# thrill/thrill

Hardware: AMD Instinct MI355X
Metric: TeraSort keys/sec (100-byte recs) (higher is better)
Workload: dtype u8; 1 GPU; terasort_10GiB_100B; records=107374182, record_bytes=100, seed=0x7421, parallelism=dp1

## Files before the change

thrill_amd/csrc/t9_bitonic.h:

```cpp
#pragma once
#include "t9_common.h"

__device__ inline void t9_ce_xor(u64& c, u32& v, u32 lanemask, bool lower,
                                 bool asc) {
    const u64 oc = __shfl_xor(c, lanemask);
    const u32 ov = __shfl_xor(v, lanemask);
    if ((c > oc) == (lower == asc)) { c = oc; v = ov; }
}

template <int SUBMAX, int BLOCK, bool HAS_VAL>
__global__ __launch_bounds__(BLOCK, 2) void k_bitonic_sort_sub(
    u64* __restrict__ keys, u32* __restrict__ vals,
    const u32* __restrict__ sub_start, const u32* __restrict__ sub_n) {
    constexpr int E = SUBMAX / BLOCK;
    static_assert(E == 4, "mapping assumes 4 elements per thread");
    __shared__ u64 s_c[SUBMAX];
    __shared__ u32 s_v[HAS_VAL ? SUBMAX : 1];
    __shared__ u32 s_differ;

    const u32 sb = blockIdx.x;
    const u32 ns = sub_n[sb];
    if (ns <= 1 || ns > (u32)SUBMAX) return;
    const u32 gbase = sub_start[sb];
    const u32 tid = threadIdx.x, lane = tid & 63;

    if (tid == 0) s_differ = 0;
    __syncthreads();

    const u64 mask48 = 0x0000FFFFFFFFFFFFull;
    const u64 high16 = keys[gbase] & ~mask48;
    const u64 ref48 = keys[gbase] & mask48;

    u64 c[E];
    u32 v[E];
    u32 differ = 0;
    const u32 e0 = tid * E;
#pragma unroll
    for (int r = 0; r < E; ++r) {
        const u32 i = e0 + r;
        if (i < ns) {
            const u64 k = keys[gbase + i];
            c[r] = ((k & mask48) << 12) | (u64)i;
            if (HAS_VAL) v[r] = vals[gbase + i];
            differ |= ((k & mask48) != ref48);
        } else {
            c[r] = ~0ull;
            if (HAS_VAL) v[r] = 0;
        }
    }
    if (differ) s_differ = 1;
    __syncthreads();
    if (!s_differ) return;

    constexpr int LOG = (SUBMAX == 1024) ? 10 : (SUBMAX == 2048) ? 11 : 12;
// ... 39 lines not shown
                        const bool asc = ((e0 + r) & k) == 0;
                        if ((c[r] > c[q]) == asc) {
                            u64 tc = c[r]; c[r] = c[q]; c[q] = tc;
                            if (HAS_VAL) {
                                u32 tv = v[r]; v[r] = v[q]; v[q] = tv;
                            }
                        }
                    }
                }
            }
        }
    }

#pragma unroll
    for (int r = 0; r < E; ++r) {
        const u32 i = e0 + r;
        if (i < ns) {
            keys[gbase + i] = high16 | (c[r] >> 12);
            if (HAS_VAL) vals[gbase + i] = v[r];
        }
    }
}

typedef unsigned long long t9_u64x2 __attribute__((ext_vector_type(2)));

__device__ __forceinline__ u32 t9_w16_phys(u32 e) {
    return e ^ (((e >> 4) & 7u) << 1);
}

__device__ __forceinline__ void t9_w16_row_store(u64* lc, u32 row,
                                                 const u64 (&c)[16]) {
    const u32 base = row * 16 + ((row & 7u) << 1);
#pragma unroll
    for (int k = 0; k < 8; ++k) {
        t9_u64x2 v2;
        v2.x = c[2 * k];
        v2.y = c[2 * k + 1];
        *(t9_u64x2*)&lc[base ^ ((u32)k << 1)] = v2;
    }
}

__device__ __forceinline__ void t9_w16_row_load(const u64* lc, u32 row,
                                                u64 (&c)[16]) {
    const u32 base = row * 16 + ((row & 7u) << 1);
#pragma unroll
    for (int k = 0; k < 8; ++k) {
        const t9_u64x2 v2 = *(const t9_u64x2*)&lc[base ^ ((u32)k << 1)];
        c[2 * k] = v2.x;
        c[2 * k + 1] = v2.y;
    }
}

template <int NSORT, int BLOCK, bool HAS_VAL, bool REC>
__global__ __launch_bounds__(BLOCK, 2) void k_wave16_sort_sub(
    u64* __restrict__ keys, u32* __restrict__ vals,
    const u32* __restrict__ sub_start, const u32* __restrict__ sub_n,
    u32* __restrict__ ntied) {
    constexpr int E = NSORT / BLOCK;
    static_assert(E == 16, "wave16 mapping: 16 elements per lane");
    static_assert(HAS_VAL || !REC, "the tie count rides the pair sort");
    constexpr int ROUNDS = (NSORT == 1024) ? 6 : (NSORT == 2048) ? 7 : 8;
    __shared__ __attribute__((aligned(16))) u64 lc[NSORT];
    __shared__ u32 s_differ;
    __shared__ u32 s_ntie;

    const u32 sb = blockIdx.x;
    const u32 ns = sub_n[sb];
    if (ns <= 1 || ns > (u32)NSORT) return;
    const u32 gbase = sub_start[sb];
    const u32 lane = threadIdx.x;
    const u32 e0 = lane * E;

    if (lane == 0) { s_differ = 0; s_ntie = 0; }
    __syncthreads();

    const u64 mask48 = 0x0000FFFFFFFFFFFFull;
    const u64 high16 = keys[gbase] & ~mask48;
    const u64 ref48 = keys[gbase] & mask48;

    u64 c[E];
    u32 differ = 0;
    u64* const kb = keys + gbase;
    u32* const vb = HAS_VAL ? vals + gbase : nullptr;
#pragma unroll
    for (int r = 0; r < E; ++r) {
        const u32 p = lane + (u32)BLOCK * r;
        u64 cc = ~0ull;
        if (p < ns) {
            const u64 k = kb[p];
            cc = ((k & mask48) << 12) | (u64)p;
            differ |= ((k & mask48) != ref48);
        }
        lc[t9_w16_phys(p)] = cc;
    }
    if (differ) s_differ = 1;
    __syncthreads();
    if (!s_differ) {
        if (REC && lane == 0) atomicAdd(ntied, ns - 1);
        return;
    }
    t9_w16_row_load(lc, lane, c);

#pragma unroll
    for (int lk = 1; lk <= 4; ++lk) {
        const int k = 1 << lk;
#pragma unroll
        for (int lj = lk - 1; lj >= 0; --lj) {
            const int j = 1 << lj;
#pragma unroll
            for (int r = 0; r < E; ++r) {
                const int q = r ^ j;
                if (q > r) {
                    const bool asc = (r & k) == 0;
                    if ((c[r] > c[q]) == asc) {
                        u64 tc = c[r]; c[r] = c[q]; c[q] = tc;
                    }
                }
            }
        }
// ... 30 lines not shown
                ia += ta ? 1u : 0u;
                ib += ta ? 0u : 1u;
                const u32 nx = ta ? ia : ib;
                const bool in = nx < (ta ? ea : eb);
                const u64 ld = lc[t9_w16_phys(in ? nx : ab)];
                const u64 nv = in ? ld : ~0ull;
                a = ta ? nv : a;
                b = ta ? b : nv;
            }
        }
    }

    __syncthreads();
    t9_w16_row_store(lc, lane, c);
    __syncthreads();
    if (REC) {
        const u64 nxt = (e0 + E < (u32)NSORT) ? lc[t9_w16_phys(e0 + E)]
                                              : ~0ull;
        u32 cnt = 0;
#pragma unroll
        for (int r = 0; r < E; ++r) {
            const u64 hi = (r + 1 < E) ? c[r + 1] : nxt;
            cnt += (e0 + r + 1 < ns) && ((c[r] >> 12) == (hi >> 12));
        }
        if (cnt) atomicAdd(&s_ntie, cnt);
    }
    u32 v[HAS_VAL ? E : 1];
    if (HAS_VAL) {
#pragma unroll
        for (int r = 0; r < E; ++r) {
            const u32 p = lane + (u32)BLOCK * r;
            if (p < ns) v[r] = vb[(u32)lc[t9_w16_phys(p)] & 0xFFFu];
        }
    }
    __syncthreads();
    const u32 nt = REC ? s_ntie : 0u;
    if (REC && lane == 0 && nt) atomicAdd(ntied, nt);
    if (HAS_VAL) {
#pragma unroll
        for (int r = 0; r < E; ++r) {
            const u32 p = lane + (u32)BLOCK * r;
            if (p < ns) vb[p] = v[r];
        }
    }
    if (!REC || nt) {
#pragma unroll
        for (int r = 0; r < E; ++r) {
            const u32 p = lane + (u32)BLOCK * r;
            if (p < ns) kb[p] = high16 | (lc[t9_w16_phys(p)] >> 12);
        }
    }
}

template <int NSORT, int BLOCK, bool HAS_VAL>
__global__ __launch_bounds__(BLOCK, 2) void k_wave16_sort_span(
    const u64* __restrict__ keys_in, const u32* __restrict__ vals_in,
    u64* __restrict__ keys_out, u32* __restrict__ vals_out,
    const u32* __restrict__ span_start, const u32* __restrict__ span_len) {
    constexpr int E = NSORT / BLOCK;
    static_assert(E == 16, "wave16 mapping: 16 elements per lane");
    constexpr int ROUNDS = (NSORT == 1024) ? 6 : (NSORT == 2048) ? 7 : 8;
    __shared__ u64 lc[NSORT];
    __shared__ u32 s_differ;

    const u32 sb = blockIdx.x;
    const u32 ns = span_len[sb];
    if (ns == 0) return;
    const u32 gbase = span_start[sb];
    const u32 lane = threadIdx.x;
    const u32 e0 = lane * E;

    if (ns > (u32)NSORT) {
        if (keys_out != keys_in)
            for (u32 i = lane; i < ns; i += BLOCK) {
                keys_out[gbase + i] = keys_in[gbase + i];
                if (HAS_VAL) vals_out[gbase + i] = vals_in[gbase + i];
            }
        return;
    }

    if (lane == 0) s_differ = 0;
    __syncthreads();

    const u64 mask48 = 0x0000FFFFFFFFFFFFull;
    const u64 high16 = keys_in[gbase] & ~mask48;
    const u64 ref48 = keys_in[gbase] & mask48;

    u64 c[E];
    u32 differ = 0;
#pragma unroll
    for (int r = 0; r < E; ++r) {
        const u32 i = e0 + r;
        if (i < ns) {
            const u64 k = keys_in[gbase + i];
            c[r] = ((k & mask48) << 12) | (u64)i;
            differ |= ((k & mask48) != ref48);
        } else {
            c[r] = ~0ull;
        }
    }
    if (differ) s_differ = 1;
    __syncthreads();
    if (!s_differ) {
        if (keys_out != keys_in) {
#pragma unroll
            for (int r = 0; r < E; ++r) {
// ... 75 lines not shown
```

thrill_amd/csrc/t9_rank_scatter.h:

```cpp
#pragma once
#include "t9_common.h"

template <int NDIG>
__device__ inline void t9_scan_onewave(u32* s_vals, u32 tid) {
    if (tid < 64) {
        const u32 lane = tid;
        u32 carry = 0;
        for (int c = 0; c < NDIG / 64; ++c) {
            const u32 v0 = s_vals[c * 64 + lane];
            u32 v = v0;
            for (int off = 1; off < 64; off <<= 1) {
                u32 y = __shfl_up(v, off);
                if (lane >= (u32)off) v += y;
            }
            const u32 total = __shfl(v, 63);
            s_vals[c * 64 + lane] = (v - v0) + carry;
            carry += total;
        }
    }
}

__device__ inline void t9_scan256_onewave(u32* s_vals, u32 tid) {
    if (tid < 64) {
        const u32 lane = tid;
        u32 carry = 0;
        for (int c = 0; c < 4; ++c) {
            const u32 v0 = s_vals[c * 64 + lane];
            u32 v = v0;
            for (int off = 1; off < 64; off <<= 1) {
                u32 y = __shfl_up(v, off);
                if (lane >= (u32)off) v += y;
            }
            const u32 total = __shfl(v, 63);
            s_vals[c * 64 + lane] = (v - v0) + carry;
            carry += total;
        }
    }
}

template <int BITS>
__device__ inline void t9_hist_ballot_add(u32* __restrict__ s_cnt, u32 d,
                                          bool valid, u32 lane) {
    u64 m = __ballot(valid);
    for (int b = 0; b < BITS; ++b) {
        const u64 bb = __ballot((d >> b) & 1u);
        m &= ((d >> b) & 1u) ? bb : ~bb;
    }
    if (valid && (u32)__popcll(m & ((1ull << lane) - 1ull)) == 0)
        atomicAdd(&s_cnt[d], (u32)__popcll(m));
}

template <int TILE, int BLOCK, bool HAS_KEY, bool HAS_VAL,
          int REC_WORDS = 0, bool IOTA_VAL = false>
__global__ __launch_bounds__(BLOCK, 8) void k_scatter_wave512(
    const u64* __restrict__ in_keys, const u32* __restrict__ in_vals,
    u64* __restrict__ out_keys, u32* __restrict__ out_vals,
    const u32* __restrict__ offs, u64 n, u32 shift) {
    constexpr int NW = BLOCK / 64;
    constexpr int SUB = TILE / NW;
    constexpr int GROUPS = SUB / 64;
    static_assert(HAS_KEY, "the store phase reads the digit from the key");
    static_assert(TILE % BLOCK == 0 && SUB % 64 == 0, "whole groups");
    const u32* rec32 = (const u32*)in_keys;
    __shared__ __align__(16) u8 s_raw[TILE * 8];
    u64* const s_okeys = (u64*)s_raw;
    u32* const s_ovals = (u32*)s_raw;
    static_assert(TILE <= 65535, "u16 counts and offsets");
    __shared__ u16 s_wcnt[NW * T9_RADIX];
    __shared__ u32 s_start[T9_RADIX];
    __shared__ u32 s_goff[T9_RADIX];

    const u32 tid = threadIdx.x, wave = tid >> 6, lane = tid & 63;
    const u64 base = (u64)blockIdx.x * TILE;
    const u32 tn = (u32)((n - base < (u64)TILE) ? (n - base) : (u64)TILE);

    if (tid < T9_RADIX)
        s_goff[tid] = offs[(u64)blockIdx.x * T9_RADIX + tid];
    u16* const wc = s_wcnt + wave * T9_RADIX;
    for (u32 t = lane; t < T9_RADIX; t += 64) wc[t] = 0;

    u32 pos[GROUPS];
    const u32 wbase = wave * SUB;
#pragma unroll
    for (int g = 0; g < GROUPS; ++g) {
        const u32 i = wbase + g * 64 + lane;
        const bool valid = i < tn;
        u32 d = 0;
        if (valid) {
            if (REC_WORDS)
                d = ((const u8*)rec32)[(base + i) * (u64)REC_WORDS * 4 +
                                       (7 - shift / 8)];
            else
                d = (u32)(in_keys[base + i] >> shift) & 255u;
        }
        u64 m = __ballot(valid);
        for (int bit = 0; bit < 8; ++bit) {
            u64 bb = __ballot((d >> bit) & 1u);
            m &= ((d >> bit) & 1u) ? bb : ~bb;
        }
        const u32 wr = (u32)__popcll(m & ((1ull << lane) - 1ull));
        const u32 before = valid ? (u32)wc[d] : 0;
        pos[g] = before + wr;
        if (valid && wr == 0) wc[d] = (u16)(before + (u32)__popcll(m));
    }
    __syncthreads();

    if (tid < T9_RADIX) {
        u32 run = 0;
        for (int w = 0; w < NW; ++w) {
            const u32 c = s_wcnt[w * T9_RADIX + tid];
            s_wcnt[w * T9_RADIX + tid] = (u16)run;
            run += c;
        }
        s_start[tid] = run;
    }
    __syncthreads();
    t9_scan256_onewave(s_start, tid);
    __syncthreads();

    constexpr bool LOAD_VAL = HAS_VAL && !REC_WORDS && !IOTA_VAL;
    u32 val[LOAD_VAL ? GROUPS : 1];
#pragma unroll
    for (int g = 0; g < GROUPS; ++g) {
        const u32 i = wbase + g * 64 + lane;
        if (i < tn) {
            u64 k;
            if (REC_WORDS) {
                const u64 w0 = (u64)rec32[(base + i) * REC_WORDS];
                const u64 w1 = (u64)rec32[(base + i) * REC_WORDS + 1];
                k = ((u64)__builtin_bswap32((u32)w0) << 32) |
// ... 44 lines not shown
```

thrill_amd/csrc/t9_sort_msb.hip:

```cpp

#include "t9_common.h"
#include "t9_rank_scatter.h"
#include "t9_bitonic.h"

#include <cstdlib>
#include <vector>

#define T9_MSB_TILE 8192
#define T9_SUBMAX 4096
#define T9_MSB_MIN (1u << 22)

__global__ void k_colsum(const u32*, u64, u32*);
__global__ void k_chunkscan(u32*, u64, u32*);
__global__ void k_finaloffs(u32*, u64, const u32*, const u32*);
__global__ void k_grp_scan(u32*, u64, u64*);

extern "C" void t9i_launch_hist_seg9(u32, void*, const u64*, const u32*,
                                     const u32*, u32*);
extern "C" void t9i_launch_seg_scan9(u32, void*, u32*, const u32*,
                                     const u32*, const u32*, u32*, u32*);
extern "C" void t9i_launch_scatter_seg9(u32, int, void*, const u64*,
                                        const u32*, const u32*, const u32*,
                                        u64*, u32*, const u32*);
constexpr u64 NSUB9 = 256ull * 512;
// ... 485 lines not shown
                       dim3((u32)((want < 4096) ? want : 4096)), dim3(256),
                       0, s, d_keys, cnt, d_scratch);
    u32 f = 1;
    if (hipMemcpyAsync(&f, d_scratch, 4, hipMemcpyDeviceToHost, s) !=
        hipSuccess)
        return true;
    if (hipStreamSynchronize(s) != hipSuccess) return true;
    return f != 0;
}

__global__ __launch_bounds__(256) void k_subinfo(
    const u32* __restrict__ sub_n, u32 nsub, u32 hardmax, u32 list_cap,
    u32* __restrict__ info, u32* __restrict__ list) {
    __shared__ u32 s_max;
    if (threadIdx.x == 0) s_max = 0;
    __syncthreads();
    const u32 i = blockIdx.x * 256 + threadIdx.x;
    if (i < nsub) {
        const u32 v = sub_n[i];
        atomicMax(&s_max, v);
        if (v > hardmax) {
            u32 pos = atomicAdd(&info[1], 1u);
            if (pos < list_cap) list[pos] = i;
        }
    }
    __syncthreads();
    if (threadIdx.x == 0 && s_max) atomicMax(&info[0], s_max);
}

static bool t9i_lds_wave16() {
    static const bool on = [] {
        const char* e = getenv("T9_LDS_WAVE16");
        return !(e && e[0] == '0');
    }();
    return on;
}

static u32 t9i_wave16_max() {
    static const u32 v = [] {
        const char* e = getenv("T9_WAVE16_MAX");
        return e ? (u32)atoi(e) : 1024u;
    }();
    return v;
}

static bool t9i_span_wave16() {
    static const bool on = [] {
        const char* e = getenv("T9_SPAN_WAVE16");
        return !(e && e[0] == '0');
    }();
    return on;
}

template <bool HAS_VAL, bool REC>
static void t9i_launch_wave16_sub_t(u32 grid, u32 maxsub, hipStream_t s,
                                    u64* d_keys, u32* d_vals,
                                    const u32* sub_start, const u32* sub_n,
                                    u32* d_ntied) {
    if (maxsub <= 1024)
        hipLaunchKernelGGL((k_wave16_sort_sub<1024, 64, HAS_VAL, REC>),
                           dim3(grid), dim3(64), 0, s, d_keys, d_vals,
                           sub_start, sub_n, d_ntied);
    else if (maxsub <= 2048)
        hipLaunchKernelGGL((k_wave16_sort_sub<2048, 128, HAS_VAL, REC>),
                           dim3(grid), dim3(128), 0, s, d_keys, d_vals,
                           sub_start, sub_n, d_ntied);
    else
        hipLaunchKernelGGL((k_wave16_sort_sub<4096, 256, HAS_VAL, REC>),
                           dim3(grid), dim3(256), 0, s, d_keys, d_vals,
                           sub_start, sub_n, d_ntied);
}

template <bool HAS_VAL>
static void t9i_launch_wave16_sub(u32 grid, u32 maxsub, hipStream_t s,
                                  u64* d_keys, u32* d_vals,
                                  const u32* sub_start, const u32* sub_n,
                                  u32* d_ntied = nullptr) {
    if constexpr (HAS_VAL) {
        if (d_ntied) {
            t9i_launch_wave16_sub_t<true, true>(grid, maxsub, s, d_keys,
                                                d_vals, sub_start, sub_n,
                                                d_ntied);
            return;
        }
    }
    t9i_launch_wave16_sub_t<HAS_VAL, false>(grid, maxsub, s, d_keys, d_vals,
                                            sub_start, sub_n, nullptr);
}

static bool t9i_lds_bitonic() {
    static const bool on = [] {
        const char* e = getenv("T9_LDS_BITONIC");
        return e && e[0] == '1';
    }();
    return on;
}

template <bool HAS_VAL>
static void t9i_launch_bitonic_sub(u32 grid, u32 maxsub, hipStream_t s,
                                   u64* d_keys, u32* d_vals,
                                   const u32* sub_start, const u32* sub_n) {
    if (maxsub <= 1024)
        hipLaunchKernelGGL((k_bitonic_sort_sub<1024, 256, HAS_VAL>),
                           dim3(grid), dim3(256), 0, s, d_keys, d_vals,
                           sub_start, sub_n);
    else if (maxsub <= 2048)
        hipLaunchKernelGGL((k_bitonic_sort_sub<2048, 512, HAS_VAL>),
                           dim3(grid), dim3(512), 0, s, d_keys, d_vals,
                           sub_start, sub_n);
    else
        hipLaunchKernelGGL((k_bitonic_sort_sub<4096, 1024, HAS_VAL>),
                           dim3(grid), dim3(1024), 0, s, d_keys, d_vals,
                           sub_start, sub_n);
}

template <int SUBMAX, int BLOCK, bool HAS_VAL>
__global__ __launch_bounds__(BLOCK, 4) void k_lds_sort_sub(
    u64* __restrict__ keys, u32* __restrict__ vals,
    const u32* __restrict__ sub_start, const u32* __restrict__ sub_n) {
    constexpr int NW = BLOCK / 64;
    constexpr int SUBQ = SUBMAX / NW;
    constexpr int GROUPS = SUBQ / 64;
    __shared__ u64 s_k[2][SUBMAX];
    __shared__ u32 s_v[2][HAS_VAL ? SUBMAX : 1];
    __shared__ u16 s_rank[SUBMAX];
    __shared__ u32 s_wcnt[NW * T9_RADIX];
    __shared__ u32 s_woff[NW * T9_RADIX];
    __shared__ u32 s_start[T9_RADIX];
    __shared__ u32 s_differ;

    const u32 sb = blockIdx.x;
    const u32 ns = sub_n[sb];
    if (ns <= 1 || ns > (u32)SUBMAX) return;
    const u32 gbase = sub_start[sb];
    const u32 tid = threadIdx.x, wave = tid >> 6, lane = tid & 63;

    if (tid == 0) s_differ = 0;
    __syncthreads();
    const u64 mask48 = 0x0000FFFFFFFFFFFFull;
    u64 k0ref = keys[gbase] & mask48;
// ... 144 lines not shown
                    s_wcnt[wave * T9_RADIX + d] = before + (u32)__popcll(m);
            }
        }
        __syncthreads();
        if (tid < T9_RADIX) {
            u32 run = 0;
            for (int w = 0; w < NW; ++w) {
                s_woff[w * T9_RADIX + tid] = run;
                run += s_wcnt[w * T9_RADIX + tid];
            }
            s_start[tid] = run;
        }
        __syncthreads();
        t9_scan256_onewave(s_start, tid);
        __syncthreads();
        if (tid < T9_RADIX) {
            const u32 excl = s_start[tid];
            for (int w = 0; w < NW; ++w) s_woff[w * T9_RADIX + tid] += excl;
        }
        __syncthreads();
        for (int g = 0; g < GROUPS; ++g) {
            const u32 i = wbase + g * 64 + lane;
            if (i < ns) {
                const u64 k = s_k[cur][i];
                const u32 d = (u32)(k >> shift) & 255u;
                const u32 pos = s_woff[wave * T9_RADIX + d] + s_rank[i];
                s_k[cur ^ 1][pos] = k;
                if (HAS_VAL) s_v[cur ^ 1][pos] = s_v[cur][i];
            }
        }
        __syncthreads();
        cur ^= 1;
    }
    for (u32 i = tid; i < ns; i += BLOCK) {
        keys_out[gbase + i] = s_k[cur][i];
        if (HAS_VAL) vals_out[gbase + i] = s_v[cur][i];
    }
}

namespace {
struct MsbWs {
    u64* alt_k;
    u32* alt_v;
    u32* hist;
    u32* chunkpart;
    u32* digit_base;
    u32* true_base;
    u32* abase;
    u32* bucket_n;
    u32* sub_start;
    u32* sub_n;
    u32* ovr;
    u32* span;
    u32* bp;
    u64* d_total;
    u32* sub3_start;
    u32* sub3_n;
    u32* span3;
    u64 B1, B2max;
};

constexpr u64 NSUB3 = 256ull * 256 * 256;

constexpr u32 NSUB = 256 * 256;

MsbWs carve_msb(char* p, u64 n) {
    MsbWs w;
    const u64 npad = n + 256ull * T9_MSB_TILE;
    w.B1 = t9_ceil_div(n, T9_MSB_TILE);
    w.B2max = t9_ceil_div(n, T9_MSB_TILE) + 256;
    {
        const char* l3c = getenv("T9_MSB_LEVELS");
        if (n >= T9_L3_MIN || (l3c && atoi(l3c) == 3))
            w.B2max = t9_ceil_div(n, T9_MSB_TILE) + NSUB;
        if (pass2_bits() == 9) w.B2max *= 2;
    }
    w.alt_k = (u64*)p;
    p += t9_align256(npad * 8);
    w.alt_v = (u32*)p;
    p += t9_align256(npad * 4);
    w.hist = (u32*)p;
    p += t9_align256(w.B2max * T9_RADIX * 4);
    w.chunkpart = (u32*)p;
    p += t9_align256(t9_ceil_div(w.B2max, T9_SCAN_CHUNK) * T9_RADIX * 4);
    w.digit_base = (u32*)p;
    p += t9_align256(T9_RADIX * 4);
    w.true_base = (u32*)p;
    p += t9_align256(T9_RADIX * 4);
    w.abase = (u32*)p;
    p += t9_align256(257 * 4);
    w.bucket_n = (u32*)p;
    p += t9_align256(T9_RADIX * 4);
    w.sub_start = (u32*)p;
    p += t9_align256(NSUB9 * 4);
    w.sub_n = (u32*)p;
    p += t9_align256(NSUB9 * 4);
    w.ovr = (u32*)p;
    p += t9_align256((u64)(NSUB + 2) * 4);
    w.span = (u32*)p;
    p += t9_align256((u64)(2 * (NSUB + 64) + 1) * 4);
    const char* l3 = getenv("T9_MSB_LEVELS");
    if (n >= T9_L3_MIN || (l3 && atoi(l3) == 3)) {
        w.bp = (u32*)p;
        p += t9_align256((u64)(NSUB + 1) * 4);
        w.d_total = (u64*)p;
        p += 256;
        w.sub3_start = (u32*)p;
        p += t9_align256(NSUB3 * 4);
        w.sub3_n = (u32*)p;
        p += t9_align256(NSUB3 * 4);
        w.span3 = (u32*)p;
        p += t9_align256((2 * (NSUB3 + 64) + 1) * 4);
    }
    return w;
}

u64 msb_ws_bytes(u64 n) {
    const u64 npad = n + 256ull * T9_MSB_TILE;
    const char* l3e = getenv("T9_MSB_LEVELS");
    u64 B2max = t9_ceil_div(n, T9_MSB_TILE) + 256;
    if (n >= T9_L3_MIN || (l3e && atoi(l3e) == 3))
        B2max = t9_ceil_div(n, T9_MSB_TILE) + NSUB;
    if (pass2_bits() == 9) B2max *= 2;
    u64 l3 = 0;
    if (n >= T9_L3_MIN || (l3e && atoi(l3e) == 3))
        l3 = t9_align256((u64)(NSUB + 1) * 4) + 256 +
             2 * t9_align256(NSUB3 * 4) +
             t9_align256((2 * (NSUB3 + 64) + 1) * 4);
    return l3 + t9_align256(npad * 8) + t9_align256(npad * 4) +
           t9_align256(B2max * T9_RADIX * 4) +
           t9_align256(t9_ceil_div(B2max, T9_SCAN_CHUNK) * T9_RADIX * 4) +
           4 * t9_align256(T9_RADIX * 4) + t9_align256(257 * 4) +
           2 * t9_align256(NSUB9 * 4) +
           t9_align256((u64)(NSUB + 2) * 4) +
           t9_align256((u64)(2 * (NSUB + 64) + 1) * 4);
}
}

extern "C" u64 t9i_sort_pairs_msb_workspace(u64 n) { return msb_ws_bytes(n); }

extern "C" int t9i_overlap_init(t9_context* ctx);
extern "C" int t9i_gather_chunk(const u8*, const u32*, u64, u64, u8*,
                                const u32*, hipStream_t);

#define T9_OVERLAP_K 8

static u32 overlap_chunks() {
    const char* on = getenv("T9_SORT_OVERLAP");
    if (!on || on[0] == '0' || on[0] == '\0') return 0;
    const char* e = getenv("T9_SORT_OVERLAP_CHUNKS");
    int k = e ? atoi(e) : T9_OVERLAP_K;
    if (k < 1) k = 1;
    if (k > T9_OVERLAP_MAXK) k = T9_OVERLAP_MAXK;
    return (u32)k;
}

__global__ __launch_bounds__(64) void k_chunk_bounds(
    const u32* __restrict__ sub_start, u32 nsub, u32 K,
    const u32* __restrict__ info, u32* __restrict__ out) {
    const u32 c = threadIdx.x;
    if (c < 2) out[c] = info[c];
    if (c >= 1 && c < K)
        out[1 + c] = sub_start[(u64)c * nsub / K];
}

template <bool HAS_VAL, int RW = 0>
static int sort_msb_impl(t9_context* ctx, const u64* pass1_src,
                         u64* d_keys, u32* d_vals, u64 n,
                         void* d_workspace, void* stream,
                         bool pre_hist = false,
                         t9_overlap_req* ov = nullptr,
                         bool iota_vals = false,
                         u32* d_ntied = nullptr,
                         int* tie_counted = nullptr) {
    hipStream_t s = (hipStream_t)stream;
    MsbWs w = carve_msb((char*)d_workspace, n);

    {
        const u64 B = w.B1;
        const u64 Bc = t9_ceil_div(B, T9_SCAN_CHUNK);
        if (!pre_hist)
            T9_PERF_WRAP(s, "hist_pairs",
                         hipLaunchKernelGGL((k_hist_msb<RW>), dim3((u32)B),
                                            dim3(256), 0, s, pass1_src, n,
                                            56, w.hist));
        hipLaunchKernelGGL(k_colsum, dim3((u32)Bc), dim3(256), 0, s, w.hist,
                           B, w.chunkpart);
        hipLaunchKernelGGL(k_chunkscan, dim3(1), dim3(256), 0, s,
// ... 38 lines not shown
                                                 w.bucket_n, d_keys,
                                                 d_vals, w.hist));
            T9_LAUNCH_CHECK();
            HIP_TRY(hipMemsetAsync(w.ovr, 0, 8, s));
            hipLaunchKernelGGL(k_subinfo, dim3((u32)(NSUB9 / 256)),
                               dim3(256), 0, s, w.sub_n, (u32)NSUB9,
                               T9_SUBMAX, NSUB, w.ovr, w.ovr + 2);
            const u32 K = (HAS_VAL && ov && ctx && !t9perf_on() &&
                           t9i_lds_wave16())
                              ? overlap_chunks() : 0;
            u32 info[2 + T9_OVERLAP_MAXK] = { 0, 0 };
            if (K) {
                hipLaunchKernelGGL(k_chunk_bounds, dim3(1), dim3(64), 0, s,
                                   w.sub_start, (u32)NSUB9, K, w.ovr,
                                   w.span);
                HIP_TRY(hipMemcpyAsync(info, w.span, (K + 1) * 4,
                                       hipMemcpyDeviceToHost, s));
            }
            else
                HIP_TRY(hipMemcpyAsync(info, w.ovr, 8,
                                       hipMemcpyDeviceToHost, s));
            HIP_TRY(hipStreamSynchronize(s));
            const u32 maxsub = info[0], novr9 = info[1];
            u32* tcount = nullptr;
            if constexpr (HAS_VAL) {
                if (d_ntied && novr9 == 0 &&
                    t9i_lds_wave16() && maxsub <= t9i_wave16_max()) {
                    tcount = d_ntied;
                    HIP_TRY(hipMemsetAsync(tcount, 0, 4, s));
                    if (tie_counted) *tie_counted = 1;
                }
            }
            if (K && tcount) {
                u64 bnd[T9_OVERLAP_MAXK + 1];
                bnd[0] = 0;
                bnd[K] = n;
                bool mono = true;
                for (u32 c = 1; c < K; ++c) {
                    bnd[c] = info[1 + c];
                    mono = mono && bnd[c] >= bnd[c - 1] && bnd[c] <= n;
                }
                if (mono) {
                    int rc = t9i_overlap_init(ctx);
                    if (rc) return rc;
                    hipStream_t sb = ctx->ov_stream;
                    u32 done = 0;
                    for (u32 c = 0; c < K; ++c) {
                        const u64 a = bnd[c], b = bnd[c + 1];
                        if (a == b) continue;
                        const u32 sub0 = (u32)((u64)c * NSUB9 / K);
                        const u32 sub1 = (u32)((u64)(c + 1) * NSUB9 / K);
                        t9i_launch_wave16_sub<HAS_VAL>(
                            sub1 - sub0, maxsub, s, d_keys, d_vals,
                            w.sub_start + sub0, w.sub_n + sub0, tcount);
                        T9_LAUNCH_CHECK();
                        HIP_TRY(hipEventRecord(ctx->ov_ev[c], s));
                        HIP_TRY(hipStreamWaitEvent(sb, ctx->ov_ev[c], 0));
                        rc = t9i_gather_chunk(
                            ov->recs, d_vals + a, b - a, n,
                            ov->out + a * (u64)ov->rec_words * 4,
                            tcount, sb);
                        if (rc) return rc;
                        ++done;
                    }
                    HIP_TRY(hipEventRecord(ctx->ov_ev[T9_OVERLAP_MAXK], sb));
                    HIP_TRY(hipStreamWaitEvent(
                        s, ctx->ov_ev[T9_OVERLAP_MAXK], 0));
                    ov->chunks = done;
                    return T9_OK;
                }
            }
            T9_PERF_WRAP(
                s, "lds_sort",
                if (t9i_lds_wave16() && maxsub <= t9i_wave16_max())
                    t9i_launch_wave16_sub<HAS_VAL>((u32)NSUB9, maxsub, s,
                                                   d_keys, d_vals,
                                                   w.sub_start, w.sub_n,
                                                   tcount);
                else if (t9i_lds_bitonic())
                    t9i_launch_bitonic_sub<HAS_VAL>((u32)NSUB9, maxsub, s,
                                                    d_keys, d_vals,
                                                    w.sub_start, w.sub_n);
                else if (maxsub <= 1024)
                    hipLaunchKernelGGL(
                        (k_lds_sort_sub<1024, 256, HAS_VAL>), dim3(NSUB9),
                        dim3(256), 0, s, d_keys, d_vals, w.sub_start,
                        w.sub_n);
                else if (maxsub <= 2048)
                    hipLaunchKernelGGL(
                        (k_lds_sort_sub<2048, 512, HAS_VAL>), dim3(NSUB9),
                        dim3(512), 0, s, d_keys, d_vals, w.sub_start,
                        w.sub_n);
                else
                    hipLaunchKernelGGL(
                        (k_lds_sort_sub<T9_SUBMAX, 1024, HAS_VAL>),
                        dim3(NSUB9), dim3(1024), 0, s, d_keys, d_vals,
                        w.sub_start, w.sub_n));
            T9_LAUNCH_CHECK();
            if (novr9 == 0) return T9_OK;
            if (novr9 > 64)
                return HAS_VAL ? t9i_sort_pairs_lsd(ctx, d_keys, d_vals, n,
                                                    d_workspace, stream)
                               : t9i_sort_keys_lsd(ctx, d_keys, n,
                                                   d_workspace, stream);
            std::vector<u32> list9(novr9), st9(novr9), cn9(novr9);
            HIP_TRY(hipMemcpy(list9.data(), w.ovr + 2, novr9 * 4,
                              hipMemcpyDeviceToHost));
            for (u32 i = 0; i < novr9; ++i) {
                HIP_TRY(hipMemcpy(&st9[i], w.sub_start + list9[i], 4,
                                  hipMemcpyDeviceToHost));
                HIP_TRY(hipMemcpy(&cn9[i], w.sub_n + list9[i], 4,
                                  hipMemcpyDeviceToHost));
            }
            for (u32 i = 0; i < novr9; ++i) {
                if (!range_differs(d_keys + st9[i], cn9[i], w.ovr, s))
                    continue;
                int rc = HAS_VAL
                             ? t9i_sort_pairs_lsd(ctx, d_keys + st9[i],
                                                  d_vals + st9[i], cn9[i],
                                                  d_workspace, stream)
                             : t9i_sort_keys_lsd(ctx, d_keys + st9[i],
                                                 cn9[i], d_workspace,
                                                 stream);
                if (rc) return rc;
            }
            return T9_OK;
        }
    }

    {
        const u64 B2 = w.B2max;
// ... 116 lines not shown
                                             d_workspace, stream);
            if (rc) return rc;
        }
        return T9_OK;
    }

    const char* se = getenv("T9_LDS_SPAN");
    const bool use_span = se && atoi(se) == 1;
    const u32* sel_start;
    const u32* sel_n;
    u32 novr = 0;
    if (use_span) {
        const u32 CAP = NSUB + 64;
        u32* span_count = w.span;
        u32* span_start = w.span + 1;
        u32* span_len = w.span + 1 + CAP;
        HIP_TRY(hipMemsetAsync(w.span, 0, (u64)(2 * CAP + 1) * 4, s));
        hipLaunchKernelGGL(k_span_pack, dim3(1), dim3(256), 0, s,
                           w.sub_start, w.sub_n, T9_SUBMAX, span_count,
                           span_start, span_len);
        HIP_TRY(hipMemsetAsync(w.ovr, 0, 8, s));
        hipLaunchKernelGGL(k_subinfo, dim3(CAP / 256 + 1), dim3(256), 0, s,
                           span_len, CAP, T9_SUBMAX, NSUB, w.ovr,
                           w.ovr + 2);
        u32 info[2] = { 0, 0 };
        HIP_TRY(hipMemcpyAsync(info, w.ovr, 8, hipMemcpyDeviceToHost, s));
        HIP_TRY(hipStreamSynchronize(s));
        novr = info[1];
        T9_PERF_WRAP(
            s, "lds_sort",
            hipLaunchKernelGGL(
                (k_lds_sort_span<T9_SUBMAX, 1024, HAS_VAL, 7>),
                dim3(CAP), dim3(1024), 0, s, d_keys, d_vals, d_keys,
                d_vals, span_start, span_len));
        T9_LAUNCH_CHECK();
        sel_start = span_start;
        sel_n = span_len;
    }
    else {
        HIP_TRY(hipMemsetAsync(w.ovr, 0, 8, s));
        hipLaunchKernelGGL(k_subinfo, dim3(NSUB / 256), dim3(256), 0, s,
                           w.sub_n, NSUB, T9_SUBMAX, NSUB, w.ovr,
                           w.ovr + 2);
        u32 info[2] = { 0, 0 };
        HIP_TRY(hipMemcpyAsync(info, w.ovr, 8, hipMemcpyDeviceToHost, s));
        HIP_TRY(hipStreamSynchronize(s));
        const u32 maxsub = info[0];
        novr = info[1];
        T9_PERF_WRAP(
            s, "lds_sort",
            if (t9i_lds_wave16() && maxsub <= t9i_wave16_max())
                t9i_launch_wave16_sub<HAS_VAL>((u32)NSUB, maxsub, s,
                                               d_keys, d_vals,
                                               w.sub_start, w.sub_n);
            else if (t9i_lds_bitonic())
                t9i_launch_bitonic_sub<HAS_VAL>((u32)NSUB, maxsub, s,
                                                d_keys, d_vals,
                                                w.sub_start, w.sub_n);
            else if (maxsub <= 2048)
                hipLaunchKernelGGL((k_lds_sort_sub<2048, 512, HAS_VAL>),
                                   dim3(NSUB), dim3(512), 0, s, d_keys,
                                   d_vals, w.sub_start, w.sub_n);
            else
                hipLaunchKernelGGL(
                    (k_lds_sort_sub<T9_SUBMAX, 1024, HAS_VAL>), dim3(NSUB),
                    dim3(1024), 0, s, d_keys, d_vals, w.sub_start,
                    w.sub_n));
        T9_LAUNCH_CHECK();
        sel_start = w.sub_start;
        sel_n = w.sub_n;
    }
    if (novr == 0) return T9_OK;

    if (novr > 64) {
        return HAS_VAL ? t9i_sort_pairs_lsd(ctx, d_keys, d_vals, n,
                                            d_workspace, stream)
                       : t9i_sort_keys_lsd(ctx, d_keys, n, d_workspace,
                                           stream);
    }
    HIP_TRY(hipStreamSynchronize(s));
    std::vector<u32> list(novr);
    HIP_TRY(hipMemcpy(list.data(), w.ovr + 2, novr * 4,
                      hipMemcpyDeviceToHost));
    std::vector<u32> starts(novr), counts(novr);
    for (u32 i = 0; i < novr; ++i) {
        HIP_TRY(hipMemcpy(&starts[i], sel_start + list[i], 4,
                          hipMemcpyDeviceToHost));
        HIP_TRY(hipMemcpy(&counts[i], sel_n + list[i], 4,
                          hipMemcpyDeviceToHost));
    }
    for (u32 i = 0; i < novr; ++i) {
        if (!range_differs(d_keys + starts[i], counts[i], w.ovr, s))
            continue;
        int rc = HAS_VAL
                     ? t9i_sort_pairs_lsd(ctx, d_keys + starts[i],
                                          d_vals + starts[i], counts[i],
                                          d_workspace, stream)
                     : t9i_sort_keys_lsd(ctx, d_keys + starts[i],
                                         counts[i], d_workspace, stream);
        if (rc) return rc;
    }
    return T9_OK;
}

extern "C" int t9i_sort_pairs_msb(t9_context* ctx, u64* d_keys,
                                  u32* d_vals, u64 n, void* d_workspace,
                                  void* stream) {
    return sort_msb_impl<true>(ctx, d_keys, d_keys, d_vals, n, d_workspace,
                               stream);
}

extern "C" int t9i_sort_pairs_msb_ph(t9_context* ctx, u64* d_keys,
                                     u32* d_vals, u64 n,
                                     void* d_workspace, void* stream,
                                     int iota_vals, t9_overlap_req* ov,
                                     u32* d_ntied, int* tie_counted) {
    if (tie_counted) *tie_counted = 0;
    return sort_msb_impl<true>(ctx, d_keys, d_keys, d_vals, n, d_workspace,
                               stream, true, ov, iota_vals != 0, d_ntied,
                               tie_counted);
}

extern "C" u32* t9i_msb_pass1_hist(void* d_workspace, u64 n) {
    MsbWs w = carve_msb((char*)d_workspace, n);
    return w.hist;
}

extern "C" int t9i_sort_keys_msb(t9_context* ctx, u64* d_keys, u64 n,
                                 void* d_workspace, void* stream) {
    return sort_msb_impl<false>(ctx, d_keys, d_keys, nullptr, n,
                                d_workspace, stream);
}

extern "C" int t9i_sort_recs_msb(t9_context* ctx, const u8* d_recs,
                                 u32 rec_size, u64* d_keys, u32* d_vals,
                                 u64 n, void* d_workspace, void* stream) {
    const u32 rw = rec_size / 4;
    if (rw == 25)
        return sort_msb_impl<true, 25>(ctx, (const u64*)d_recs, d_keys,
                                       d_vals, n, d_workspace, stream);
    if (rw == 32)
        return sort_msb_impl<true, 32>(ctx, (const u64*)d_recs, d_keys,
                                       d_vals, n, d_workspace, stream);
    return T9_EINVAL;
}
```

Before: 9.270 billion keys/s.

## Add narrow 32-bit wave16 subsort with redo fallback and XCD-aware scatter tile mapping

Adds a 64-lane subsort kernel for buckets of up to 1024 keys. It packs 22 distinguishing key bits plus a 10-bit index into one u32 and sorts them with a DPP/permlane bitonic network, which halves LDS and register traffic compared with the 64-bit path. Buckets where the truncated prefixes could be ambiguous are appended to a redo list and re-sorted by the existing full wave16 kernel, run as a persistent grid-stride loop. Separately, the scatter kernel remaps blockIdx so that each XCD handles a contiguous range of tiles, which should improve L2 locality. The cost is an extra launch, a memset and a gather pass through the original keys and values.

```diff
diff --git a/thrill_amd/csrc/t9_bitonic.h b/thrill_amd/csrc/t9_bitonic.h
--- a/thrill_amd/csrc/t9_bitonic.h
+++ b/thrill_amd/csrc/t9_bitonic.h
@@ -1,5 +1,6 @@
 #pragma once
 #include "t9_common.h"
+#include "t9_w16_network.h"
 
 __device__ inline void t9_ce_xor(u64& c, u32& v, u32 lanemask, bool lower,
                                  bool asc) {
@@ -145,19 +146,16 @@
 }
 
 template <int NSORT, int BLOCK, bool HAS_VAL, bool REC>
-__global__ __launch_bounds__(BLOCK, 2) void k_wave16_sort_sub(
+__device__ __forceinline__ void t9_wave16_sort_one(
     u64* __restrict__ keys, u32* __restrict__ vals,
     const u32* __restrict__ sub_start, const u32* __restrict__ sub_n,
-    u32* __restrict__ ntied) {
+    u32* __restrict__ ntied, const u32 sb, u64* lc, u32& s_differ,
+    u32& s_ntie) {
     constexpr int E = NSORT / BLOCK;
     static_assert(E == 16, "wave16 mapping: 16 elements per lane");
     static_assert(HAS_VAL || !REC, "the tie count rides the pair sort");
     constexpr int ROUNDS = (NSORT == 1024) ? 6 : (NSORT == 2048) ? 7 : 8;
-    __shared__ __attribute__((aligned(16))) u64 lc[NSORT];
-    __shared__ u32 s_differ;
-    __shared__ u32 s_ntie;
-
-    const u32 sb = blockIdx.x;
+
     const u32 ns = sub_n[sb];
     if (ns <= 1 || ns > (u32)NSORT) return;
     const u32 gbase = sub_start[sb];
@@ -294,6 +292,201 @@
     }
 }
 
+template <int NSORT, int BLOCK, bool HAS_VAL, bool REC, bool LIST = false>
+__global__ __launch_bounds__(BLOCK, 2) void k_wave16_sort_sub(
+    u64* __restrict__ keys, u32* __restrict__ vals,
+    const u32* __restrict__ sub_start, const u32* __restrict__ sub_n,
+    u32* __restrict__ ntied, const u32* __restrict__ redo_list,
+    const u32* __restrict__ redo_count) {
+    __shared__ __attribute__((aligned(16))) u64 lc[NSORT];
+    __shared__ u32 s_differ;
+    __shared__ u32 s_ntie;
+    if constexpr (!LIST) {
+        t9_wave16_sort_one<NSORT, BLOCK, HAS_VAL, REC>(
+            keys, vals, sub_start, sub_n, ntied, blockIdx.x, lc, s_differ,
+            s_ntie);
+    } else {
+        const u32 cnt = *redo_count;
+        for (u32 i = blockIdx.x; i < cnt; i += gridDim.x) {
+            t9_wave16_sort_one<NSORT, BLOCK, HAS_VAL, REC>(
+                keys, vals, sub_start, sub_n, ntied, redo_list[i], lc,
+                s_differ, s_ntie);
+            __syncthreads();
+        }
+    }
+}
+
+typedef u32 t9_u32x4 __attribute__((ext_vector_type(4)));
+
+__device__ __forceinline__ u32 t9_n16_swz(u32 row) {
+    return (((row >> 1) & 3u) ^ (((row >> 3) & 1u) * 3u)) << 2;
+}
+__device__ __forceinline__ u32 t9_n16_phys(u32 e) {
+    return e ^ t9_n16_swz(e >> 4);
+}
+
+struct t9_n16_wave {
+    typedef u32 V;
+    u32 lane;
+    __device__ __forceinline__ V cmin(V a, V b) { return a < b ? a : b; }
+    __device__ __forceinline__ V cmax(V a, V b) { return a < b ? b : a; }
+    template <int CTRL>
+    __device__ __forceinline__ V dpp(V v) {
+        if constexpr (CTRL == T9N_DPP_X1)
+            return __builtin_amdgcn_update_dpp(0u, v, 0xB1, 0xF, 0xF, true);
+        else if constexpr (CTRL == T9N_DPP_X2)
+            return __builtin_amdgcn_update_dpp(0u, v, 0x4E, 0xF, 0xF, true);
+        else if constexpr (CTRL == T9N_DPP_X3)
+            return __builtin_amdgcn_update_dpp(0u, v, 0x1B, 0xF, 0xF, true);
+        else if constexpr (CTRL == T9N_DPP_X4) {
+            const V t =
+                __builtin_amdgcn_update_dpp(0u, v, 0x104, 0xF, 0x5, false);
+            return __builtin_amdgcn_update_dpp(t, v, 0x114, 0xF, 0xA, false);
+        } else if constexpr (CTRL == T9N_DPP_X7)
+            return __builtin_amdgcn_update_dpp(0u, v, 0x141, 0xF, 0xF, true);
+        else if constexpr (CTRL == T9N_DPP_X8)
+            return __builtin_amdgcn_update_dpp(0u, v, 0x128, 0xF, 0xF, true);
+        else
+            return __builtin_amdgcn_update_dpp(0u, v, 0x140, 0xF, 0xF, true);
+    }
+    template <int D>
+    __device__ __forceinline__ V sel(V lo, V hi) {
+        return (lane & (u32)D) ? hi : lo;
+    }
+    __device__ __forceinline__ void swap16(V& a, V& b) {
+        const auto r = __builtin_amdgcn_permlane16_swap(a, b, false, false);
+        a = r[0];
+        b = r[1];
+    }
+    __device__ __forceinline__ void swap32(V& a, V& b) {
+        const auto r = __builtin_amdgcn_permlane32_swap(a, b, false, false);
+        a = r[0];
+        b = r[1];
+    }
+    template <int SEL>
+    __device__ __forceinline__ V cpl(V v) {
+        return ((t9n_cpl_mask(SEL) >> lane) & 1ull) ? ~v : v;
+    }
+};
+
+template <bool HAS_VAL, bool REC>
+__global__ __launch_bounds__(64) void k_wave16_sort_narrow(
+    u64* __restrict__ keys, u32* __restrict__ vals,
+    const u32* __restrict__ sub_start, const u32* __restrict__ sub_n,
+    u32* __restrict__ ntied,
+    u32* __restrict__ redo ) {
+    constexpr int E = 16, BLOCK = 64, NSORT = 1024;
+    static_assert(HAS_VAL || !REC, "the tie count rides the pair sort");
+    __shared__ __attribute__((aligned(16))) u32 lc[NSORT];
+    __shared__ u32 s_or[2];
+
+    const u32 sb = blockIdx.x;
+    const u32 ns = sub_n[sb];
+    if (ns <= 1 || ns > (u32)NSORT) return;
+    const u32 gbase = sub_start[sb];
+    const u32 lane = threadIdx.x;
+    const u32 e0 = lane * E;
+
+    if (lane == 0) { s_or[0] = 0; s_or[1] = 0; }
+    __syncthreads();
+
+    u64* const kb = keys + gbase;
+    u32* const vb = HAS_VAL ? vals + gbase : nullptr;
+    const u64 k0 = kb[0];
+    u64 k[E];
+    u64 orv = 0;
+#pragma unroll
+    for (int r = 0; r < E; ++r) {
+        const u32 p = lane + (u32)BLOCK * r;
+        k[r] = (p < ns) ? kb[p] : k0;
+        orv |= k[r] ^ k0;
+    }
+    if ((u32)orv) atomicOr(&s_or[0], (u32)orv);
+    if ((u32)(orv >> 32)) atomicOr(&s_or[1], (u32)(orv >> 32));
+    __syncthreads();
+    const u32 or_lo = s_or[0], or_hi = s_or[1];
+    if ((or_lo | or_hi) == 0) {
+        if (REC && lane == 0) atomicAdd(ntied, ns - 1);
+        return;
+    }
+    const u32 hb = or_hi ? 63u - (u32)__builtin_clz(or_hi)
+                         : 31u - (u32)__builtin_clz(or_lo);
+    const u32 sh = hb > 21u ? hb - 21u : 0u;
+
+#pragma unroll
+    for (int r = 0; r < E; ++r) {
+        const u32 p = lane + (u32)BLOCK * r;
+        const u32 cc = (p < ns)
+            ? ((((u32)(k[r] >> sh)) & 0x3FFFFFu) << 10) | p
+            : 0xFFFFFFFFu;
+        lc[t9_n16_phys(p)] = cc;
+    }
+    __syncthreads();
+    u32 c[E];
+    {
+        const u32 base = e0 + t9_n16_swz(lane);
+#pragma unroll
+        for (int q = 0; q < 4; ++q) {
+            const t9_u32x4 v4 = *(const t9_u32x4*)&lc[base ^ ((u32)q << 2)];
+            c[4 * q] = v4.x;
+            c[4 * q + 1] = v4.y;
+            c[4 * q + 2] = v4.z;
+            c[4 * q + 3] = v4.w;
+        }
+    }
+
+    t9_n16_wave x = { lane };
+    t9n_net<t9_n16_wave>::sort(x, c);
+
+    const u32 nxt = __shfl_down(c[0], 1);
+    u32 amb = 0;
+#pragma unroll
+    for (int r = 0; r < E; ++r) {
+        const u32 hi = (r + 1 < E) ? c[r + 1] : nxt;
+        amb |= (e0 + r + 1 < ns) && ((c[r] ^ hi) < 1024u);
+    }
+    if (__ballot(amb) != 0) {
+        if (lane == 0) redo[1 + atomicAdd(&redo[0], 1u)] = sb;
+        return;
+    }
+
+    __syncthreads();
+    {
+        const u32 base = e0 + t9_n16_swz(lane);
+#pragma unroll
+        for (int q = 0; q < 4; ++q) {
+            t9_u32x4 v4;
+            v4.x = c[4 * q];
+            v4.y = c[4 * q + 1];
+            v4.z = c[4 * q + 2];
+            v4.w = c[4 * q + 3];
+            *(t9_u32x4*)&lc[base ^ ((u32)q << 2)] = v4;
+        }
+    }
+    __syncthreads();
+    u32 v[HAS_VAL ? E : 1];
+    u64 kk[REC ? 1 : E];
+#pragma unroll
+    for (int r = 0; r < E; ++r) {
+        const u32 p = lane + (u32)BLOCK * r;
+        if (p < ns) {
+            u32 src = lc[t9_n16_phys(p)] & 1023u;
+            src = src < ns ? src : ns - 1;
+            if (HAS_VAL) v[r] = vb[src];
+            if (!REC) kk[r] = kb[src];
+        }
+    }
+    __syncthreads();
+#pragma unroll
+    for (int r = 0; r < E; ++r) {
+        const u32 p = lane + (u32)BLOCK * r;
+        if (p < ns) {
+            if (HAS_VAL) vb[p] = v[r];
+            if (!REC) kb[p] = kk[r];
+        }
+    }
+}
+
 template <int NSORT, int BLOCK, bool HAS_VAL>
 __global__ __launch_bounds__(BLOCK, 2) void k_wave16_sort_span(
     const u64* __restrict__ keys_in, const u32* __restrict__ vals_in,
diff --git a/thrill_amd/csrc/t9_rank_scatter.h b/thrill_amd/csrc/t9_rank_scatter.h
--- a/thrill_amd/csrc/t9_rank_scatter.h
+++ b/thrill_amd/csrc/t9_rank_scatter.h
@@ -71,11 +71,15 @@
     __shared__ u32 s_goff[T9_RADIX];
 
     const u32 tid = threadIdx.x, wave = tid >> 6, lane = tid & 63;
-    const u64 base = (u64)blockIdx.x * TILE;
+    const u32 xper = gridDim.x >> 3, xrem = gridDim.x & 7;
+    const u32 xcd = blockIdx.x & 7;
+    const u32 tile = xcd * xper + (xcd < xrem ? xcd : xrem) +
+                     (blockIdx.x >> 3);
+    const u64 base = (u64)tile * TILE;
     const u32 tn = (u32)((n - base < (u64)TILE) ? (n - base) : (u64)TILE);
 
     if (tid < T9_RADIX)
-        s_goff[tid] = offs[(u64)blockIdx.x * T9_RADIX + tid];
+        s_goff[tid] = offs[(u64)tile * T9_RADIX + tid];
     u16* const wc = s_wcnt + wave * T9_RADIX;
     for (u32 t = lane; t < T9_RADIX; t += 64) wc[t] = 0;
 
diff --git a/thrill_amd/csrc/t9_sort_msb.hip b/thrill_amd/csrc/t9_sort_msb.hip
--- a/thrill_amd/csrc/t9_sort_msb.hip
+++ b/thrill_amd/csrc/t9_sort_msb.hip
@@ -561,40 +561,62 @@
     return on;
 }
 
+static bool t9i_wave16_narrow() {
+    static const bool on = [] {
+        const char* e = getenv("T9_WAVE16_NARROW");
+        return !(e && e[0] == '0');
+    }();
+    return on;
+}
+
+#define T9_REDO_GRID 8192u
+
 template <bool HAS_VAL, bool REC>
 static void t9i_launch_wave16_sub_t(u32 grid, u32 maxsub, hipStream_t s,
                                     u64* d_keys, u32* d_vals,
                                     const u32* sub_start, const u32* sub_n,
-                                    u32* d_ntied) {
-    if (maxsub <= 1024)
+                                    u32* d_ntied, u32* redo) {
+    const u32* const nolist = nullptr;
+    if (maxsub <= 1024 && redo && t9i_wave16_narrow() &&
+        hipMemsetAsync(redo, 0, 4, s) == hipSuccess) {
+        hipLaunchKernelGGL((k_wave16_sort_narrow<HAS_VAL, REC>), dim3(grid),
+                           dim3(64), 0, s, d_keys, d_vals, sub_start, sub_n,
+                           d_ntied, redo);
+        hipLaunchKernelGGL((k_wave16_sort_sub<1024, 64, HAS_VAL, REC, true>),
+                           dim3(grid < T9_REDO_GRID ? grid : T9_REDO_GRID),
+                           dim3(64), 0, s, d_keys, d_vals, sub_start, sub_n,
+                           d_ntied, (const u32*)(redo + 1),
+                           (const u32*)redo);
+    }
+    else if (maxsub <= 1024)
         hipLaunchKernelGGL((k_wave16_sort_sub<1024, 64, HAS_VAL, REC>),
                            dim3(grid), dim3(64), 0, s, d_keys, d_vals,
-                           sub_start, sub_n, d_ntied);
+                           sub_start, sub_n, d_ntied, nolist, nolist);
     else if (maxsub <= 2048)
         hipLaunchKernelGGL((k_wave16_sort_sub<2048, 128, HAS_VAL, REC>),
                            dim3(grid), dim3(128), 0, s, d_keys, d_vals,
-                           sub_start, sub_n, d_ntied);
+                           sub_start, sub_n, d_ntied, nolist, nolist);
     else
         hipLaunchKernelGGL((k_wave16_sort_sub<4096, 256, HAS_VAL, REC>),
                            dim3(grid), dim3(256), 0, s, d_keys, d_vals,
-                           sub_start, sub_n, d_ntied);
+                           sub_start, sub_n, d_ntied, nolist, nolist);
 }
 
 template <bool HAS_VAL>
 static void t9i_launch_wave16_sub(u32 grid, u32 maxsub, hipStream_t s,
                                   u64* d_keys, u32* d_vals,
                                   const u32* sub_start, const u32* sub_n,
-                                  u32* d_ntied = nullptr) {
+                                  u32* redo, u32* d_ntied = nullptr) {
     if constexpr (HAS_VAL) {
         if (d_ntied) {
             t9i_launch_wave16_sub_t<true, true>(grid, maxsub, s, d_keys,
                                                 d_vals, sub_start, sub_n,
-                                                d_ntied);
+                                                d_ntied, redo);
             return;
         }
     }
     t9i_launch_wave16_sub_t<HAS_VAL, false>(grid, maxsub, s, d_keys, d_vals,
-                                            sub_start, sub_n, nullptr);
+                                            sub_start, sub_n, nullptr, redo);
 }
 
 static bool t9i_lds_bitonic() {
@@ -845,6 +867,7 @@
     u32* sub_n;
     u32* ovr;
     u32* span;
+    u32* redo;
     u32* bp;
     u64* d_total;
     u32* sub3_start;
@@ -892,6 +915,8 @@
     p += t9_align256((u64)(NSUB + 2) * 4);
     w.span = (u32*)p;
     p += t9_align256((u64)(2 * (NSUB + 64) + 1) * 4);
+    w.redo = (u32*)p;
+    p += t9_align256((NSUB9 + 1) * 4);
     const char* l3 = getenv("T9_MSB_LEVELS");
     if (n >= T9_L3_MIN || (l3 && atoi(l3) == 3)) {
         w.bp = (u32*)p;
@@ -926,7 +951,8 @@
            4 * t9_align256(T9_RADIX * 4) + t9_align256(257 * 4) +
            2 * t9_align256(NSUB9 * 4) +
            t9_align256((u64)(NSUB + 2) * 4) +
-           t9_align256((u64)(2 * (NSUB + 64) + 1) * 4);
+           t9_align256((u64)(2 * (NSUB + 64) + 1) * 4) +
+           t9_align256((NSUB9 + 1) * 4);
 }
 }
 
@@ -1071,7 +1097,8 @@
                         const u32 sub1 = (u32)((u64)(c + 1) * NSUB9 / K);
                         t9i_launch_wave16_sub<HAS_VAL>(
                             sub1 - sub0, maxsub, s, d_keys, d_vals,
-                            w.sub_start + sub0, w.sub_n + sub0, tcount);
+                            w.sub_start + sub0, w.sub_n + sub0, w.redo,
+                            tcount);
                         T9_LAUNCH_CHECK();
                         HIP_TRY(hipEventRecord(ctx->ov_ev[c], s));
                         HIP_TRY(hipStreamWaitEvent(sb, ctx->ov_ev[c], 0));
@@ -1095,7 +1122,7 @@
                     t9i_launch_wave16_sub<HAS_VAL>((u32)NSUB9, maxsub, s,
                                                    d_keys, d_vals,
                                                    w.sub_start, w.sub_n,
-                                                   tcount);
+                                                   w.redo, tcount);
                 else if (t9i_lds_bitonic())
                     t9i_launch_bitonic_sub<HAS_VAL>((u32)NSUB9, maxsub, s,
                                                     d_keys, d_vals,
@@ -1318,7 +1345,8 @@
             if (t9i_lds_wave16() && maxsub <= t9i_wave16_max())
                 t9i_launch_wave16_sub<HAS_VAL>((u32)NSUB, maxsub, s,
                                                d_keys, d_vals,
-                                               w.sub_start, w.sub_n);
+                                               w.sub_start, w.sub_n,
+                                               w.redo);
             else if (t9i_lds_bitonic())
                 t9i_launch_bitonic_sub<HAS_VAL>((u32)NSUB, maxsub, s,
                                                 d_keys, d_vals,
@@ -1392,6 +1420,11 @@
     return w.hist;
 }
 
+extern "C" u32* t9i_msb_redo_list(void* d_workspace, u64 n) {
+    MsbWs w = carve_msb((char*)d_workspace, n);
+    return w.redo;
+}
+
 extern "C" int t9i_sort_keys_msb(t9_context* ctx, u64* d_keys, u64 n,
                                  void* d_workspace, void* stream) {
     return sort_msb_impl<false>(ctx, d_keys, d_keys, nullptr, n,
diff --git a/thrill_amd/csrc/t9_w16_network.h b/thrill_amd/csrc/t9_w16_network.h
--- /dev/null
+++ b/thrill_amd/csrc/t9_w16_network.h
@@ -0,0 +1,144 @@
+#pragma once
+#include <stdint.h>
+
+#if defined(__HIPCC__)
+#define T9N_FN __host__ __device__ __forceinline__
+#else
+#define T9N_FN inline
+#endif
+
+enum {
+    T9N_DPP_X1 = 0,
+    T9N_DPP_X2,
+    T9N_DPP_X3,
+    T9N_DPP_X4,
+    T9N_DPP_X7,
+    T9N_DPP_X8,
+    T9N_DPP_X15
+};
+
+enum {
+    T9N_CPL_L4 = 0,
+    T9N_CPL_L4X5,
+    T9N_CPL_L5
+};
+
+constexpr uint64_t t9n_cpl_mask(int sel) {
+    return sel == T9N_CPL_L4     ? 0xFFFF0000FFFF0000ull
+           : sel == T9N_CPL_L4X5 ? 0x0000FFFFFFFF0000ull
+                                 : 0xFFFFFFFF00000000ull;
+}
+
+constexpr uint64_t t9n_lower_mask(int d) {
+    uint64_t m = 0;
+    for (int l = 0; l < 64; ++l)
+        if ((l & d) == 0) m |= 1ull << l;
+    return m;
+}
+
+struct t9n_stage {
+    int lk, lj;
+    int flip;
+    int medium;
+    uint64_t lower;
+    int cpl_before;
+};
+
+constexpr t9n_stage t9n_stage_at(int s) {
+    int lk = 1, lj = 0;
+    for (int i = 0; i < s; ++i) {
+        if (lj > 0) --lj;
+        else { ++lk; lj = lk - 1; }
+    }
+    t9n_stage st = { lk, lj, (lk <= 8 && lj == lk - 1) ? 1 : 0,
+                     lj < 4 ? 0 : lj < 8 ? 1 : lj == 8 ? 2 : 3,
+                     lj < 4 ? 0ull : t9n_lower_mask(1 << (lj - 4)),
+                     (lk == 1)               ? T9N_CPL_L4
+                     : (lk == 9 && lj == 8)  ? T9N_CPL_L4X5
+                     : (lk == 10 && lj == 9) ? T9N_CPL_L5
+                                             : -1 };
+    return st;
+}
+constexpr int T9N_STAGES = 55;
+
+template <class X>
+struct t9n_net {
+    typedef typename X::V V;
+
+    static T9N_FN void ce(X& x, V& a, V& b) {
+        const V lo = x.cmin(a, b), hi = x.cmax(a, b);
+        a = lo;
+        b = hi;
+    }
+
+    template <int LK, int LJ>
+    static T9N_FN void stage(X& x, V (&c)[16]) {
+        constexpr bool first = (LJ == LK - 1);
+        constexpr bool flip = first && LK <= 8;
+        if constexpr (LK == 1) {
+#pragma unroll
+            for (int r = 0; r < 16; ++r)
+                c[r] = x.template cpl<T9N_CPL_L4>(c[r]);
+        }
+        if constexpr (LK == 9 && LJ == 8) {
+#pragma unroll
+            for (int r = 0; r < 16; ++r)
+                c[r] = x.template cpl<T9N_CPL_L4X5>(c[r]);
+        }
+        if constexpr (LK == 10 && LJ == 9) {
+#pragma unroll
+            for (int r = 0; r < 16; ++r)
+                c[r] = x.template cpl<T9N_CPL_L5>(c[r]);
+        }
+        if constexpr (LJ < 4) {
+            constexpr int j = 1 << LJ;
+            constexpr int px = flip ? ((1 << LK) - 1) : j;
+#pragma unroll
+            for (int r = 0; r < 16; ++r)
+                if ((r & j) == 0) ce(x, c[r], c[r ^ px]);
+        } else if constexpr (LJ < 8) {
+            constexpr int d = 1 << (LJ - 4);
+            constexpr int ctrl =
+                flip ? (d == 1 ? T9N_DPP_X1 : d == 2 ? T9N_DPP_X3
+                        : d == 4 ? T9N_DPP_X7 : T9N_DPP_X15)
+                     : (d == 1 ? T9N_DPP_X1 : d == 2 ? T9N_DPP_X2
+                        : d == 4 ? T9N_DPP_X4 : T9N_DPP_X8);
+            if constexpr (flip) {
+#pragma unroll
+                for (int r = 0; r < 8; ++r) {
+                    const V pa = x.template dpp<ctrl>(c[r ^ 15]);
+                    const V pb = x.template dpp<ctrl>(c[r]);
+                    c[r] = x.template sel<d>(x.cmin(c[r], pa),
+                                             x.cmax(c[r], pa));
+                    c[r ^ 15] = x.template sel<d>(x.cmin(c[r ^ 15], pb),
+                                                  x.cmax(c[r ^ 15], pb));
+                }
+            } else {
+#pragma unroll
+                for (int r = 0; r < 16; ++r) {
+                    const V p = x.template dpp<ctrl>(c[r]);
+                    c[r] = x.template sel<d>(x.cmin(c[r], p),
+                                             x.cmax(c[r], p));
+                }
+            }
+        } else {
+#pragma unroll
+            for (int r = 0; r < 16; r += 2) {
+                if constexpr (LJ == 8) x.swap16(c[r], c[r + 1]);
+                else x.swap32(c[r], c[r + 1]);
+                ce(x, c[r], c[r + 1]);
+                if constexpr (LJ == 8) x.swap16(c[r], c[r + 1]);
+                else x.swap32(c[r], c[r + 1]);
+            }
+        }
+    }
+
+    template <int LK, int LJ>
+    static T9N_FN void from(X& x, V (&c)[16]) {
+        stage<LK, LJ>(x, c);
+        if constexpr (LJ > 0) from<LK, LJ - 1>(x, c);
+        else if constexpr (LK < 10) from<LK + 1, LK>(x, c);
+    }
+
+    static T9N_FN void sort(X& x, V (&c)[16]) { from<1, 0>(x, c); }
+};
```

Result: faster. 9.549 billion keys/s, median of 6 (+3.0%).
